# tphakala/birda

Hardware: AMD Instinct MI355X
Metric: 3s/48kHz segments/sec (BirdNET v2.4) (higher is better)
Workload: dtype f16x3; 1 GPU; configs[1]: 1000 synthetic 3 s/48 kHz segments per GPU per step, HBM-resident, seeded synthetic BirdNET-v2.4-shaped model (EfficientNet-B0-like, 6522 classes); segments_per_gpu=1000, micro_batch=1000, fused_blocks=16, precision=auto

## Files before the change

birda_amd/csrc/kernels_conv.hip:

```cpp
#include "kernels.hpp"

namespace bh {

typedef float f32x4 __attribute__((ext_vector_type(4)));

__device__ __forceinline__ float act_apply(float v, int act) { return act_apply_slow(v, act); }

constexpr int PW_BK = 32;

template <int BM, int NT, bool GATE = false>
__global__ __launch_bounds__(256) void pw_gemm_kernel(const float *__restrict__ A, const float *__restrict__ W,
                                                       const float *__restrict__ bias, const float *__restrict__ R,
                                                       float *__restrict__ C, int M, int K, int N, int ldw, int act,
                                                       const float *__restrict__ gate = nullptr, int rows_per_seg = 1, int res_after = 0) {
    constexpr int BN = NT * 16;
    constexpr int WM = BM / 4;
    constexpr int MT = WM / 16;
    constexpr int AS = PW_BK + 4;
    constexpr int BS = BN + 4;
    constexpr int A4 = BM * PW_BK / 4 / 256;
    constexpr int B4 = (PW_BK * BN / 4 + 255) / 256;
    __shared__ __attribute__((aligned(16))) float As[2][BM * AS];
    __shared__ __attribute__((aligned(16))) float Bs[2][PW_BK * BS];

// ... 255 lines not shown
    const int li = lane & 15, kq = lane >> 4;
    const int t0 = ((int)blockIdx.x * 4 + wave) * NT;
    if (t0 >= n_tiles) return;
    const int steps = K / 32;
    f32x4 acc[NT];
#pragma unroll
    for (int j = 0; j < NT; j++) acc[j] = (f32x4){0.f, 0.f, 0.f, 0.f};
    const float *arow = A + (size_t)min(li, M - 1) * K + 8 * kq;
    float4 ra[PF][2];
    f16x8 bh[PF][NT], bl[PF][NT];
    auto load = [&](int st, float4 (&a)[2], f16x8 (&h)[NT], f16x8 (&l)[NT]) {
        a[0] = *reinterpret_cast<const float4 *>(arow + 32 * st);
        a[1] = *reinterpret_cast<const float4 *>(arow + 32 * st + 4);
#pragma unroll
        for (int j = 0; j < NT; j++) {
            const int t = min(t0 + j, n_tiles - 1);
            h[j] = Wf[(((size_t)st * n_tiles + t) * BH_PL(TERMS) + 0) * 64 + lane];
            if (TERMS == 3) l[j] = Wf[(((size_t)st * n_tiles + t) * 2 + 1) * 64 + lane];
        }
    };
#pragma unroll
    for (int u = 0; u < PF; u++)
        if (u < steps) load(u, ra[u], bh[u], bl[u]);
    for (int st0 = 0; st0 < steps; st0 += PF) {
#pragma unroll
        for (int u = 0; u < PF; u++) {
            const int st = st0 + u;
            if (st < steps) {
                const float v[8] = {ra[u][0].x, ra[u][0].y, ra[u][0].z, ra[u][0].w, ra[u][1].x, ra[u][1].y, ra[u][1].z, ra[u][1].w};
                f16x8 ah, al;
                bh_split8(v, ah, al);
#pragma unroll
                for (int j = 0; j < NT; j++) {
                    acc[j] = __builtin_amdgcn_mfma_f32_16x16x32_f16(ah, bh[u][j], acc[j], 0, 0, 0);
                    if (TERMS == 3) acc[j] = __builtin_amdgcn_mfma_f32_16x16x32_f16(ah, bl[u][j], acc[j], 0, 0, 0);
                    if (TERMS >= 2) acc[j] = __builtin_amdgcn_mfma_f32_16x16x32_f16(al, bh[u][j], acc[j], 0, 0, 0);
                }
                if (st + PF < steps) load(st + PF, ra[u], bh[u], bl[u]);
            }
        }
    }
#pragma unroll
    for (int j = 0; j < NT; j++) {
        const int col = (t0 + j) * 16 + li;
        if (col >= N) continue;
        const float bv = bias[col];
#pragma unroll
        for (int r = 0; r < 4; r++) {
            const int row = kq * 4 + r;
            if (row < M) {
                float v = __builtin_fmaf(acc[j][r], w_unscale, bv);
                if constexpr (AFTER) v = bh_act_after<ACT>(v + R[(size_t)row * N + col]);
                else { v = bh_act<ACT>(v); if (R) v += R[(size_t)row * N + col]; }
                C[(size_t)row * N + col] = v;
            }
        }
    }
}

template <int TERMS, int ACT, bool GATE = false, int NTB = 8, bool BLK = false, bool AFTER = false>
__global__ __launch_bounds__(256, 2) void pw_gemm16s_kernel(const float *__restrict__ A, const f16x8 *__restrict__ Wf,
                                                            const float *__restrict__ bias, const float *__restrict__ R,
                                                            float *__restrict__ C, int M, int K, int N, int n_tiles, float w_unscale,
                                                            const float *__restrict__ gate = nullptr, int rows_per_seg = 1) {
    extern __shared__ __attribute__((aligned(16))) float gsm[];
    constexpr int STAGE = (8 + NTB) * 2 * 256;
    constexpr int NJ = NTB / 2;
    static_assert(NTB % 2 == 0 && NTB >= 2 && NTB <= 12, "column tiles per workgroup");
    static_assert(!(AFTER && GATE), "the gated project GEMMs have no after-the-add form");
    const int tid = threadIdx.x, lane = tid & 63, wave = tid >> 6;
    const int li = lane & 15, kq = lane >> 4;
    const int wm = wave >> 1, wn = wave & 1;
    const int n_xb = (n_tiles + NTB - 1) / NTB, n_yb = (M + 127) / 128;
    int yb, xb;
    if constexpr (GATE) {
        yb = (int)blockIdx.x / n_xb; xb = (int)blockIdx.x - yb * n_xb;
        if (yb >= n_yb) return;
    } else {
        const int xcd = blockIdx.x & 7, slot = blockIdx.x >> 3;
        yb = slot % n_yb; xb = (slot / n_yb) * 8 + xcd;
        if (xb >= n_xb) return;
    }
    const int mb0 = yb * 128, tb0 = xb * NTB;
    const int steps = GATE ? (K + 31) / 32 : K / 32;
    const unsigned lds0 = (__builtin_amdgcn_groupstaticsize() + 15u) & ~15u;
    const int ws = __builtin_amdgcn_readfirstlane(wave);

    const int srow = tid >> 2, skq = tid & 3;
    const float *ag[2], *gg[2];
    int adst[2];
#pragma unroll
    for (int q = 0; q < 2; q++) {
        const int row = srow + 64 * q, grow = min(mb0 + row, M - 1);
        ag[q] = BLK ? A + (size_t)(grow >> 4) * 16 * K + ((skq >> 1) * 16 + (grow & 15)) * 16 + (skq & 1) * 8 : A + (size_t)grow * K + 8 * skq;
        gg[q] = GATE ? gate + (size_t)(grow / rows_per_seg) * K + 8 * skq : nullptr;
        adst[q] = (((row >> 4) * 2) * 64 + skq * 16 + (row & 15)) * 4;
    }
    float4 ra[2][2], rg[GATE ? 2 : 1][2];
    constexpr int a_step = BLK ? 512 : 32;
    auto load_a = [&](int st) {
#pragma unroll
        for (int q = 0; q < 2; q++) {
            if constexpr (GATE) {
#pragma unroll
                for (int h = 0; h < 2; h++) {
                    const bool in = 32 * st + 8 * skq + 4 * h < K;
                    ra[q][h] = *reinterpret_cast<const float4 *>(ag[q] + (in ? a_step * st + 4 * h : 0));
                    rg[q][h] = *reinterpret_cast<const float4 *>(gg[q] + (in ? 32 * st + 4 * h : 0));
                    if (!in) { rg[q][h] = make_float4(0.f, 0.f, 0.f, 0.f); ra[q][h] = rg[q][h]; }
                }
            } else {
                ra[q][0] = *reinterpret_cast<const float4 *>(ag[q] + 32 * st);
                ra[q][1] = *reinterpret_cast<const float4 *>(ag[q] + 32 * st + 4);
            }
        }
    };
    auto store_a = [&](int buf) {
        float *as = gsm + buf * STAGE;
#pragma unroll
        for (int q = 0; q < 2; q++) {
            float v[8] = {ra[q][0].x, ra[q][0].y, ra[q][0].z, ra[q][0].w, ra[q][1].x, ra[q][1].y, ra[q][1].z, ra[q][1].w};
            if constexpr (GATE) {
                const float g[8] = {rg[q][0].x, rg[q][0].y, rg[q][0].z, rg[q][0].w, rg[q][1].x, rg[q][1].y, rg[q][1].z, rg[q][1].w};
#pragma unroll
                for (int j = 0; j < 8; j++) v[j] *= g[j];
            }
            f16x8 h, l;
            bh_split8(v, h, l);
            *reinterpret_cast<f16x8 *>(as + adst[q]) = h;
            if (TERMS >= 2) *reinterpret_cast<f16x8 *>(as + adst[q] + 256) = l;
        }
    };
    auto dma_b = [&](int st, int buf) {
#pragma unroll
        for (int jj = 0; jj < (NTB + 3) / 4; jj++) {
            const int j = ws + 4 * jj, t = min(tb0 + j, n_tiles - 1);
            if (j >= NTB) continue;
#pragma unroll
            for (int pl = 0; pl < (TERMS == 3 ? 2 : 1); pl++) {
                const f16x8 *src = Wf + (((size_t)st * n_tiles + t) * BH_PL(TERMS) + pl) * 64;
                const unsigned dst = lds0 + 4u * (unsigned)(buf * STAGE + 8 * 2 * 256 + (j * 2 + pl) * 256);
                asm volatile("s_mov_b32 m0, %2\n\ts_nop 0\n\tglobal_load_lds_dwordx4 %0, %1"
                             :: "v"((unsigned)lane * 16u), "s"(src), "s"(dst) : "memory", "m0");
            }
        }
    };

    f32x4 acc[4][NJ];
#pragma unroll
    for (int i = 0; i < 4; i++)
#pragma unroll
        for (int j = 0; j < NJ; j++) acc[i][j] = (f32x4){0.f, 0.f, 0.f, 0.f};

    dma_b(0, 0);
    load_a(0);
    store_a(0);
    asm volatile("s_waitcnt vmcnt(0)" ::: "memory");
    __syncthreads();
    for (int st = 0; st < steps; st++) {
        const int cur = st & 1;
        const bool more = st + 1 < steps;
        if (more) { dma_b(st + 1, cur ^ 1); load_a(st + 1); }
        const float *as = gsm + cur * STAGE, *bs = as + 8 * 2 * 256;
        f16x8 ah[4], al[4], bh[NJ], bl[NJ];
#pragma unroll
        for (int i = 0; i < 4; i++) {
            ah[i] = *reinterpret_cast<const f16x8 *>(as + (((wm * 4 + i) * 2) * 64 + lane) * 4);
            if (TERMS >= 2) al[i] = *reinterpret_cast<const f16x8 *>(as + (((wm * 4 + i) * 2 + 1) * 64 + lane) * 4);
        }
#pragma unroll
        for (int j = 0; j < NJ; j++) {
            bh[j] = *reinterpret_cast<const f16x8 *>(bs + (((wn * NJ + j) * 2) * 64 + lane) * 4);
            if (TERMS == 3) bl[j] = *reinterpret_cast<const f16x8 *>(bs + (((wn * NJ + j) * 2 + 1) * 64 + lane) * 4);
        }
#pragma unroll
        for (int i = 0; i < 4; i++)
#pragma unroll
            for (int j = 0; j < NJ; j++) {
                acc[i][j] = __builtin_amdgcn_mfma_f32_16x16x32_f16(ah[i], bh[j], acc[i][j], 0, 0, 0);
                if (TERMS == 3) acc[i][j] = __builtin_amdgcn_mfma_f32_16x16x32_f16(ah[i], bl[j], acc[i][j], 0, 0, 0);
                if (TERMS >= 2) acc[i][j] = __builtin_amdgcn_mfma_f32_16x16x32_f16(al[i], bh[j], acc[i][j], 0, 0, 0);
            }
        if (more) store_a(cur ^ 1);
        asm volatile("s_waitcnt vmcnt(0)" ::: "memory");
        __syncthreads();
    }
    const int m0 = mb0 + wm * 64, t0 = tb0 + wn * NJ;
#pragma unroll
    for (int j = 0; j < NJ; j++) {
        const int col = (t0 + j) * 16 + li;
        if (col >= N) continue;
        const float bv = bias[col];
#pragma unroll
        for (int i = 0; i < 4; i++)
#pragma unroll
            for (int r = 0; r < 4; r++) {
                const int row = m0 + i * 16 + kq * 4 + r;
                if (row < M) {
                    float v = __builtin_fmaf(acc[i][j][r], w_unscale, bv);
                    if constexpr (AFTER) v = bh_act_after<ACT>(v + R[(size_t)row * N + col]);
                    else { v = bh_act<ACT>(v); if (R) v += R[(size_t)row * N + col]; }
                    C[(size_t)row * N + col] = v;
                }
            }
    }
}

bool pw_gemm16_supports(int K, int act) { return K % 32 == 0 && (act == ACT_NONE || act_is_templated(act)); }
bool pw_gemm16_after_supports(int K, int act) { return K % 32 == 0 && act_is_templated_after(act); }

#define BH_LOAD_STREAM(p) (*(p))
template <int TERMS, int NT, bool SHALLOW = false, int DBG = 0>
__global__ __launch_bounds__(512, SHALLOW ? 4 : 2) void pw_gemm16_thin_kernel(const float *__restrict__ A, const float *__restrict__ gate, int rows_per_seg,
                                                                 const f16x8 *__restrict__ Wf, const float *__restrict__ bias,
                                                                 const float *__restrict__ R, float *__restrict__ C, int M, int K, int N,
                                                                 float w_unscale) {
    extern __shared__ __attribute__((aligned(16))) float tsm[];
    const int tid = threadIdx.x, lane = tid & 63, wave = tid >> 6;
    const int li = lane & 15, kq = lane >> 4;
    const int steps = (K + 31) / 32;
    {
        const float4 *src = reinterpret_cast<const float4 *>(Wf);
        float4 *dst = reinterpret_cast<float4 *>(tsm);
        const int n4 = steps * NT * BH_PL(TERMS) * 64;
        for (int i = tid; i < n4; i += 512) dst[i] = src[i];
    }
    __syncthreads();
    const f16x8 *wf = reinterpret_cast<const f16x8 *>(tsm);
    const int n_rt = (M + 15) >> 4;
    const float rcp_p = 1.0f / (float)rows_per_seg;
    constexpr int RB = SHALLOW ? (NT <= 2 ? 3 : 2) : (NT <= 2 ? 4 : 3);
    for (int rt0 = (blockIdx.x * 8 + wave) * RB; rt0 < n_rt; rt0 += gridDim.x * 8 * RB) {
        const float *ap[RB], *gp[RB];
#pragma unroll
        for (int r = 0; r < RB; r++) {
            const int row = min((rt0 + r) * 16 + li, M - 1);
            int seg = (int)((float)row * rcp_p);
            seg += (row - seg * rows_per_seg >= rows_per_seg) ? 1 : 0;
            seg -= (row - seg * rows_per_seg < 0) ? 1 : 0;
            ap[r] = A + (size_t)row * K + 8 * kq;
            gp[r] = gate + (size_t)seg * K + 8 * kq;
        }
        f32x4 acc[RB][NT];
#pragma unroll
        for (int r = 0; r < RB; r++)
#pragma unroll
            for (int j = 0; j < NT; j++) acc[r][j] = (f32x4){0.f, 0.f, 0.f, 0.f};
        float4 ra[RB][2], rg[RB][2];
        auto load = [&](int st, float4 (&a)[RB][2], float4 (&g)[RB][2]) {
#pragma unroll
            for (int r = 0; r < RB; r++)
#pragma unroll
                for (int h = 0; h < 2; h++) {
                    const bool in = 32 * st + 8 * kq + 4 * h < K;
                    a[r][h] = BH_LOAD_STREAM(reinterpret_cast<const float4 *>(ap[r] + (in ? 32 * st + 4 * h : 0)));
                    g[r][h] = *reinterpret_cast<const float4 *>(gp[r] + (in ? 32 * st + 4 * h : 0));
                    if (!in) { a[r][h] = make_float4(0.f, 0.f, 0.f, 0.f); g[r][h] = a[r][h]; }
                }
        };
        for (int st = 0; st < steps; st++) {
            load(st, ra, rg);
            f16x8 ah[RB], al[RB];
#pragma unroll
            for (int r = 0; r < RB; r++) {
                const float v[8] = {ra[r][0].x * rg[r][0].x, ra[r][0].y * rg[r][0].y, ra[r][0].z * rg[r][0].z, ra[r][0].w * rg[r][0].w,
                                    ra[r][1].x * rg[r][1].x, ra[r][1].y * rg[r][1].y, ra[r][1].z * rg[r][1].z, ra[r][1].w * rg[r][1].w};
                bh_split8(v, ah[r], al[r]);
            }
            if constexpr ((DBG & 1) != 0) {
#pragma unroll
                for (int r = 0; r < RB; r++) acc[r][0][0] += (float)ah[r][0] + (float)al[r][7];
                continue;
            }
#pragma unroll
            for (int j = 0; j < NT; j++) {
                const f16x8 bh = wf[((st * NT + j) * BH_PL(TERMS) + 0) * 64 + lane];
                f16x8 bl;
                if (TERMS == 3) bl = wf[((st * NT + j) * 2 + 1) * 64 + lane];
#pragma unroll
                for (int r = 0; r < RB; r++) {
                    acc[r][j] = __builtin_amdgcn_mfma_f32_16x16x32_f16(ah[r], bh, acc[r][j], 0, 0, 0);
                    if (TERMS == 3) acc[r][j] = __builtin_amdgcn_mfma_f32_16x16x32_f16(ah[r], bl, acc[r][j], 0, 0, 0);
                    if (TERMS >= 2) acc[r][j] = __builtin_amdgcn_mfma_f32_16x16x32_f16(al[r], bh, acc[r][j], 0, 0, 0);
                }
            }
        }
        if constexpr ((DBG & 8) != 0) {
            float t = 0.f;
#pragma unroll
            for (int r = 0; r < RB; r++)
#pragma unroll
                for (int j = 0; j < NT; j++) t += acc[r][j][0] + acc[r][j][1] + acc[r][j][2] + acc[r][j][3];
            if (t == 12345.678f) C[0] = t;
            continue;
        }
        float *ep = tsm + (size_t)steps * NT * BH_PL(TERMS) * 256 + (size_t)wave * (RB * 16 * NT * 16);
#pragma unroll
        for (int r = 0; r < RB; r++)
#pragma unroll
            for (int j = 0; j < NT; j++) {
                const int col = j * 16 + li;
                if (col >= N) continue;
                const float bv = bias[col];
#pragma unroll
                for (int q = 0; q < 4; q++) ep[(r * 16 + kq * 4 + q) * N + col] = __builtin_fmaf(acc[r][j][q], w_unscale, bv);
            }
        __builtin_amdgcn_fence(__ATOMIC_RELEASE, "wavefront");
        __builtin_amdgcn_wave_barrier();
        const int row0 = rt0 * 16, nrows = min(RB * 16, M - row0);
        const int nflt = nrows * N;
        float *cg = C + (size_t)row0 * N;
        const float *rgp = R ? R + (size_t)row0 * N : nullptr;
        for (int f = lane * 4; f < nflt; f += 256) {
            float4 v = *reinterpret_cast<const float4 *>(ep + f);
            if (rgp) { const float4 rr = *reinterpret_cast<const float4 *>(rgp + f); v.x += rr.x; v.y += rr.y; v.z += rr.z; v.w += rr.w; }
            *reinterpret_cast<float4 *>(cg + f) = v;
        }
        __builtin_amdgcn_wave_barrier();
    }
}

#define BH_GDBG(bit) ((DBG & (bit)) != 0)
template <int N_> __device__ __forceinline__ void bh_wait_vm() { asm volatile("s_waitcnt vmcnt(%0)" :: "n"(N_) : "memory"); }
template <int TERMS, int NT, int RB, int PF, int DBG = 0>
__global__ __launch_bounds__(512, 1) void pw_gemm16_wide_kernel(const float *__restrict__ A, const float *__restrict__ gate, int rows_per_seg,
                                                                 const f16x8 *__restrict__ Wf, const float *__restrict__ bias,
                                                                 const float *__restrict__ R, float *__restrict__ C, int M, int K, int N,
                                                                 float w_unscale, int gs_max, int a_blocked) {
    extern __shared__ __attribute__((aligned(16))) float wsm[];
    constexpr int PL = BH_PL(TERMS);
    constexpr int STEP_FL = NT * PL * 256;
    constexpr int PIECES = (NT * PL + 7) / 8;
    constexpr int ND = RB * 2;
    constexpr int INFLIGHT = ND + (PF - 2) * (PIECES + ND);
    static_assert(PF >= 2 && PF <= 4 && INFLIGHT <= 63, "prefetch depth");
    const int tid = threadIdx.x, lane = tid & 63, wave = tid >> 6;
    const int li = lane & 15, kq = lane >> 4;
    const int steps = (K + 31) / 32, KP = steps * 32;
    float *gs = wsm + PF * STEP_FL;
    float *ep = wsm + (size_t)wave * (16 * NT * 16);
    const int n_rt = (M + 15) >> 4;
    const float rcp_p = 1.0f / (float)rows_per_seg;
    const unsigned lds0 = (__builtin_amdgcn_groupstaticsize() + 15u) & ~15u;
    const int ws = __builtin_amdgcn_readfirstlane(wave);
    auto dma_w = [&](int st) {
        const int buf = st % PF;
#pragma unroll
        for (int i = 0; i < PIECES; i++) {
            const int p = min(ws + 8 * i, NT * PL - 1);
            const f16x8 *src = Wf + ((size_t)st * NT * PL + p) * 64;
            const unsigned dst = lds0 + 4u * (unsigned)(buf * STEP_FL + p * 256);
            asm volatile("s_mov_b32 m0, %2\n\ts_nop 0\n\tglobal_load_lds_dwordx4 %0, %1"
// ... 165 lines not shown
            asm volatile("" ::: "memory");
        }
        if constexpr (BH_GDBG(64)) {
            asm volatile("s_waitcnt vmcnt(0)" ::: "memory");
            const long long t_3 = __builtin_readcyclecounter();
            if (lane == 0) {
                long long *st = reinterpret_cast<long long *>(C + (size_t)M * N) + ((size_t)blockIdx.x * 8 + wave) * 4;
                st[0] = t_1 - t_0; st[1] = t_2 - t_1; st[2] = t_3 - t_2; st[3] = t_0;
            }
        }
    }
}

bool pw_gemm16_gated_wants_blocked(int K, int N, int rows_per_seg) {
    const int n_tiles = (N + 15) / 16;
    return K % 16 == 0 && rows_per_seg % 16 == 0 && N % 4 == 0 && n_tiles >= 6 && n_tiles <= 15;
}

const char *launch_pw_gemm16_gated(const float *A, const float *gate, int rows_per_seg, const void *Wf, const float *bias, const float *R,
                                   float *C, int M, int K, int N, int terms, float w_unscale, int a_blocked, hipStream_t s) {
    const char *name = nullptr;
    const int n_tiles = (N + 15) / 16;
    const size_t w_bytes = (size_t)((K + 31) / 32) * n_tiles * 2 * 1024;
    if (n_tiles <= 3 && w_bytes <= 64 * 1024 && M >= 4096 && N % 4 == 0 && !a_blocked) {
        const bool shallow = K <= 32;
        const size_t thin_lds = w_bytes / 2 * BH_PL(terms) + (size_t)8 * (shallow ? (n_tiles <= 2 ? 3 : 2) : (n_tiles <= 2 ? 4 : 3)) * 16 * n_tiles * 16 * sizeof(float);
        const int n_rt = (M + 15) / 16;
        const int wgs = std::min((n_rt + 31) / 32, 2 * device_cu_count());
#define BH_THIN(T, NTV, SH)                                                                                                        \
        do {                                                                                                                       \
            static DeviceOnce attr;                                                                                                \
            attr.run([] { (void)hipFuncSetAttribute((const void *)pw_gemm16_thin_kernel<T, NTV, SH>, hipFuncAttributeMaxDynamicSharedMemorySize, 128 * 1024); }); \
            hipLaunchKernelGGL((pw_gemm16_thin_kernel<T, NTV, SH>), dim3(wgs), dim3(512), thin_lds, s, A, gate, rows_per_seg, (const f16x8 *)Wf, bias, R, C, M, K, N, w_unscale); \
            name = "pw_gemm16_thin_kernel<" #T ",NT=" #NTV ",SHALLOW=" #SH ">";                                                   \
        } while (0)
#define BH_THIN_S(T, NTV) do { if (shallow) BH_THIN(T, NTV, true); else BH_THIN(T, NTV, false); } while (0)
        if (terms == 3) { if (n_tiles == 1) BH_THIN_S(3, 1); else if (n_tiles == 2) BH_THIN_S(3, 2); else BH_THIN_S(3, 3); }
        else if (terms == 2) { if (n_tiles == 1) BH_THIN_S(2, 1); else if (n_tiles == 2) BH_THIN_S(2, 2); else BH_THIN_S(2, 3); }
        else { if (n_tiles == 1) BH_THIN_S(1, 1); else if (n_tiles == 2) BH_THIN_S(1, 2); else BH_THIN_S(1, 3); }
#undef BH_THIN_S
#undef BH_THIN
        return name;
    }
    if (n_tiles >= 4 && n_tiles <= 15 && M >= (n_tiles >= 10 ? 40960 : 4096) && N % 4 == 0) {
        const int n_rt = (M + 15) / 16;
#define BH_WIDE(T, NTV, RBV, PFV)                                                                                                  \
        do {                                                                                                                       \
            const int gs_max = (8 * RBV * 16 + rows_per_seg - 2) / rows_per_seg + 1;                                              \
            const size_t lds = std::max((size_t)PFV * NTV * BH_PL(T) * 1024 + (size_t)gs_max * ((K + 31) / 32 * 32) * sizeof(float),         \
                                        (size_t)8 * 16 * NTV * 16 * sizeof(float));                                              \
            if (lds > 160 * 1024) break;                                \
            const int wgs = std::min((n_rt + 8 * RBV - 1) / (8 * RBV), device_cu_count());                                       \
            static DeviceOnce attr;                                                                                                \
            attr.run([] { (void)hipFuncSetAttribute((const void *)pw_gemm16_wide_kernel<T, NTV, RBV, PFV>, hipFuncAttributeMaxDynamicSharedMemorySize, 160 * 1024); }); \
            hipLaunchKernelGGL((pw_gemm16_wide_kernel<T, NTV, RBV, PFV>), dim3(wgs), dim3(512), lds, s, A, gate, rows_per_seg, (const f16x8 *)Wf, bias, R, C, M, K, N, w_unscale, gs_max, a_blocked); \
            return "pw_gemm16_wide_kernel<" #T ",NT=" #NTV ",RB=" #RBV ",PF=" #PFV ">";                                          \
        } while (0)
#define BH_WIDE_T(T)                                                                             \
        switch (n_tiles) {                                                                      \
        case 4: BH_WIDE(T, 4, 3, 3); break; case 5: BH_WIDE(T, 5, 3, 3); break; case 6: BH_WIDE(T, 6, 3, 3); break; case 7: BH_WIDE(T, 7, 3, 3); break; case 8: BH_WIDE(T, 8, 2, 4); break; case 9: BH_WIDE(T, 9, 2, 4); break;  \
        case 10: BH_WIDE(T, 10, 2, 3); break; case 11: BH_WIDE(T, 11, 2, 3); break; case 12: BH_WIDE(T, 12, 2, 3); break; case 13: BH_WIDE(T, 13, 2, 3); break; \
        case 14: BH_WIDE(T, 14, 2, 3); break; default: BH_WIDE(T, 15, 2, 3); break; }
        if (terms == 3) { BH_WIDE_T(3) } else if (terms == 2) { BH_WIDE_T(2) } else { BH_WIDE_T(1) }
#undef BH_WIDE_T
#undef BH_WIDE
    }
    int ntb = 8;
    {
        long best = -1;
        for (int cand : {10, 8, 6}) {
            const long padded = (long)((n_tiles + cand - 1) / cand) * cand;
            if (best < 0 || padded < best) { best = padded; ntb = cand; }
        }
    }
    const int n_xb = (n_tiles + ntb - 1) / ntb, n_yb = (M + 127) / 128;
    dim3 grid((unsigned)(n_xb * n_yb)), block(256);
#define BH_GS(T, NTBV, BLKV)                                                                                                      \
    do {                                                                                                                          \
        constexpr size_t lds = 2 * ((8 + NTBV) * 2 * 256) * sizeof(float);                                                       \
        static DeviceOnce attr;                                                                                                   \
        attr.run([] { (void)hipFuncSetAttribute((const void *)pw_gemm16s_kernel<T, ACT_NONE, true, NTBV, BLKV>, hipFuncAttributeMaxDynamicSharedMemorySize, (int)lds); }); \
        hipLaunchKernelGGL((pw_gemm16s_kernel<T, ACT_NONE, true, NTBV, BLKV>), grid, block, lds, s, A, (const f16x8 *)Wf, bias, R, C, M, K, N, n_tiles, w_unscale, gate, rows_per_seg); \
        name = "pw_gemm16s_kernel<" #T ",NONE,GATE,NTB=" #NTBV ",BLK=" #BLKV ">";                                                 \
    } while (0)
#define BH_GS_B(T, NTBV) do { if (a_blocked) BH_GS(T, NTBV, true); else BH_GS(T, NTBV, false); } while (0)
    if (terms == 3) { if (ntb == 6) BH_GS_B(3, 6); else if (ntb == 10) BH_GS_B(3, 10); else BH_GS_B(3, 8); }
    else if (terms == 2) { if (ntb == 6) BH_GS_B(2, 6); else if (ntb == 10) BH_GS_B(2, 10); else BH_GS_B(2, 8); }
    else { if (ntb == 6) BH_GS_B(1, 6); else if (ntb == 10) BH_GS_B(1, 10); else BH_GS_B(1, 8); }
#undef BH_GS_B
#undef BH_GS
    return name;
}

const char *launch_pw_gemm16(const float *A, const void *Wf, const float *bias, const float *R, float *C, int M, int K, int N,
                             int act, int terms, float w_unscale, hipStream_t s, int res_after) {
    if (res_after && (!R || !act_is_templated_after(act))) return nullptr;
    const int n_tiles = (N + 15) / 16;
    const int n_xb = (n_tiles + 7) / 8, n_yb = (M + 127) / 128;
    dim3 grid((unsigned)(8 * ((n_xb + 7) / 8) * n_yb)), block(256);
    static const bool stream_only = [] { const char *e = BH_XENV("BIRDA_HIP_GEMM_STREAM"); return e && e[0] == '1'; }();
    const bool staged = M >= 64 && !stream_only;
    const int ntb = !staged ? 8 : n_xb * n_yb >= 384 ? 8 : ((n_tiles + 3) / 4) * n_yb >= 384 ? 4 : 2;
    const int n_xb_s = (n_tiles + ntb - 1) / ntb;
    const dim3 grid_s((unsigned)(8 * ((n_xb_s + 7) / 8) * n_yb));
    const char *name = nullptr;
#define BH_G16S(T, ACTV, AN, NTBV, AFT, AFN)                                                                                      \
    do {                                                                                                                          \
        constexpr size_t lds = 2 * ((8 + NTBV) * 2 * 256) * sizeof(float);                                                        \
        static DeviceOnce attr;                                                                                                   \
        attr.run([] { (void)hipFuncSetAttribute((const void *)pw_gemm16s_kernel<T, ACTV, false, NTBV, false, AFT>, hipFuncAttributeMaxDynamicSharedMemorySize, (int)lds); }); \
        hipLaunchKernelGGL((pw_gemm16s_kernel<T, ACTV, false, NTBV, false, AFT>), grid_s, block, lds, s, A, (const f16x8 *)Wf, bias, R, C, M, K, N, n_tiles, w_unscale); \
        name = "pw_gemm16s_kernel<" #T "," AN AFN ",NTB=" #NTBV ">";                                                             \
    } while (0)
#define BH_G16(T, ACTV, AN, AFT, AFN)                                                                                             \
    do {                                                                                                                          \
        if (staged) {                                                                                                             \
            if (ntb == 8) BH_G16S(T, ACTV, AN, 8, AFT, AFN); else if (ntb == 4) BH_G16S(T, ACTV, AN, 4, AFT, AFN); else BH_G16S(T, ACTV, AN, 2, AFT, AFN); \
        } else if (M <= 32) {     \
            for (int m0 = 0; m0 < M; m0 += 16)                                                                                    \
                hipLaunchKernelGGL((pw_gemm16_skinny_kernel<T, ACTV, AFT>), dim3((unsigned)((n_tiles + 7) / 8)), block, 0, s, A + (size_t)m0 * K, (const f16x8 *)Wf, bias, \
                                   R ? R + (size_t)m0 * N : nullptr, C + (size_t)m0 * N, std::min(16, M - m0), K, N, n_tiles, w_unscale); \
            name = "pw_gemm16_skinny_kernel<" #T "," AN AFN ">";                                                                 \
        } else {                                                                                                                  \
            hipLaunchKernelGGL((pw_gemm16_kernel<T, ACTV, AFT>), grid, block, 0, s, A, (const f16x8 *)Wf, bias, R, C, M, K, N, n_tiles, w_unscale); \
            name = "pw_gemm16_kernel<" #T "," AN AFN ">";                                                                        \
        }                                                                                                                         \
    } while (0)
#define BH_G16A(T)                                                   \
    switch (act) {                                                   \
    case ACT_GELU_ERF: BH_G16(T, ACT_GELU_ERF, "GELU", false, ""); break; \
    case ACT_SWISH: BH_G16(T, ACT_SWISH, "SWISH", false, ""); break; \
    case ACT_RELU6: BH_G16(T, ACT_RELU6, "RELU6", false, ""); break; \
    case ACT_HSWISH: BH_G16(T, ACT_HSWISH, "HSWISH", false, ""); break; \
    default: BH_G16(T, ACT_NONE, "NONE", false, ""); break;          \
    }
#define BH_G16AA(T)                                                  \
    switch (act) {                                                   \
    case ACT_GELU_ERF: BH_G16(T, ACT_GELU_ERF, "GELU", true, ",AFTER"); break; \
    case ACT_SWISH: BH_G16(T, ACT_SWISH, "SWISH", true, ",AFTER"); break; \
    case ACT_RELU6: BH_G16(T, ACT_RELU6, "RELU6", true, ",AFTER"); break; \
    case ACT_HSWISH: BH_G16(T, ACT_HSWISH, "HSWISH", true, ",AFTER"); break; \
    default: BH_G16(T, ACT_RELU, "RELU", true, ",AFTER"); break;     \
    }
    if (res_after) { if (terms == 3) { BH_G16AA(3) } else if (terms == 2) { BH_G16AA(2) } else { BH_G16AA(1) } }
    else if (terms == 3) { BH_G16A(3) } else if (terms == 2) { BH_G16A(2) } else { BH_G16A(1) }
#undef BH_G16AA
#undef BH_G16A
#undef BH_G16
#undef BH_G16S
    return name;
}

template <int PT, int SW, int TERMS, int ACT, int CT = 8>
__global__ __launch_bounds__(256, 1) void head_gap16_kernel(const float *__restrict__ A, const f16x8 *__restrict__ Wf,
                                                             const float *__restrict__ bias, float *__restrict__ out,
                                                             int n_seg, int P, int K, int N, int n_tiles, int n_cb, float w_unscale) {
    constexpr int RT = PT * SW;
    constexpr int PL = BH_PL(TERMS);
    __shared__ __attribute__((aligned(16))) f16x8 Bs[2][CT * PL * 64];
    const int tid = threadIdx.x, lane = tid & 63, wave = tid >> 6;
    const int li = lane & 15, kq = lane >> 4;
    const int xcd = blockIdx.x & 7, bi = blockIdx.x >> 3;
    const int cb = bi % n_cb, mb = (bi / n_cb) * 8 + xcd;
    const int seg0 = (mb * 4 + wave) * SW;
    if (mb * 4 * SW >= n_seg) return;
    const int steps = K / 32;

    auto dma = [&](int st, int buf) {
        const f16x8 *src = Wf + ((size_t)st * n_tiles + cb * CT) * PL * 64;
#pragma unroll
        for (int q = 0; q < (CT * PL + 3) / 4; q++) {
            const int piece = q * 4 + wave;
            if (piece >= CT * PL) continue;
            const unsigned la = (unsigned)(size_t)(&Bs[buf][piece * 64]);
            asm volatile("s_mov_b32 m0, %1\n\ts_nop 0\n\tglobal_load_lds_dwordx4 %0, off"
                         :: "v"(src + piece * 64 + lane), "s"(__builtin_amdgcn_readfirstlane(la)) : "memory", "m0");
        }
    };
    int aoff[RT];
#pragma unroll
    for (int i = 0; i < RT; i++) {
        const int seg = min(seg0 + i / PT, n_seg - 1), px = min((i % PT) * 16 + li, P - 1);
        aoff[i] = (seg * P + px) * K + 8 * kq;
    }
    float4 ra[RT][2];
    auto load_a = [&](int st) {
#pragma unroll
        for (int i = 0; i < RT; i++) {
            ra[i][0] = *reinterpret_cast<const float4 *>(A + (size_t)aoff[i] + 32 * st);
            ra[i][1] = *reinterpret_cast<const float4 *>(A + (size_t)aoff[i] + 32 * st + 4);
        }
    };
    f32x4 acc[RT][CT];
#pragma unroll
    for (int j = 0; j < CT; j++)
#pragma unroll
        for (int i = 0; i < RT; i++) acc[i][j] = (f32x4){0.f, 0.f, 0.f, 0.f};
    f16x8 ah[RT], al[RT];
    auto split_a = [&]() {
#pragma unroll
        for (int i = 0; i < RT; i++) {
            const float v[8] = {ra[i][0].x, ra[i][0].y, ra[i][0].z, ra[i][0].w, ra[i][1].x, ra[i][1].y, ra[i][1].z, ra[i][1].w};
            bh_split8(v, ah[i], al[i]);
        }
    };
    auto compute = [&](int buf) {
#pragma unroll
        for (int j = 0; j < CT; j++) {
            const f16x8 bh = Bs[buf][(j * PL + 0) * 64 + lane];
            f16x8 bl;
            if (TERMS == 3) bl = Bs[buf][(j * 2 + 1) * 64 + lane];
#pragma unroll
            for (int i = 0; i < RT; i++) {
                acc[i][j] = __builtin_amdgcn_mfma_f32_16x16x32_f16(ah[i], bh, acc[i][j], 0, 0, 0);
                if (TERMS == 3) acc[i][j] = __builtin_amdgcn_mfma_f32_16x16x32_f16(ah[i], bl, acc[i][j], 0, 0, 0);
                if (TERMS >= 2) acc[i][j] = __builtin_amdgcn_mfma_f32_16x16x32_f16(al[i], bh, acc[i][j], 0, 0, 0);
            }
        }
    };
    dma(0, 0);
    load_a(0);
    asm volatile("s_waitcnt vmcnt(0)" ::: "memory");
    __syncthreads();
    for (int st = 0; st + 1 < steps; st++) {
        dma(st + 1, (st + 1) & 1);
        split_a();
        __builtin_amdgcn_sched_barrier(0);
        load_a(st + 1);
        __builtin_amdgcn_sched_barrier(0);
        compute(st & 1);
        asm volatile("s_waitcnt vmcnt(0)" ::: "memory");
        __syncthreads();
    }
    split_a();
    __builtin_amdgcn_sched_barrier(0);
    compute((steps - 1) & 1);

    const float inv_p = 1.0f / (float)P;
#pragma unroll
    for (int sg = 0; sg < SW; sg++) {
        const int seg = seg0 + sg;
#pragma unroll
        for (int j = 0; j < CT; j++) {
            float sum = 0.0f;
            const float b = bias[(cb * CT + j) * 16 + li];
#pragma unroll
            for (int t = 0; t < PT; t++) {
                const f32x4 a4 = acc[sg * PT + t][j];
                bh_f32x2 v01 = {__builtin_fmaf(a4[0], w_unscale, b), __builtin_fmaf(a4[1], w_unscale, b)},
                         v23 = {__builtin_fmaf(a4[2], w_unscale, b), __builtin_fmaf(a4[3], w_unscale, b)};
                bh_act4<ACT>(v01, v23);
                const int px = t * 16 + 4 * kq;
                if (PT * 16 == P || px + 3 < P) sum += (v01[0] + v01[1]) + (v23[0] + v23[1]);
                else sum += (px < P ? v01[0] : 0.f) + (px + 1 < P ? v01[1] : 0.f) + (px + 2 < P ? v23[0] : 0.f);
            }
            sum += __shfl_xor(sum, 16, 64);
            sum += __shfl_xor(sum, 32, 64);
            if (kq == 0 && seg < n_seg) out[(size_t)seg * N + (cb * CT + j) * 16 + li] = sum * inv_p;
        }
    }
}

bool head_gap16_supports(int P, int K, int N, int act) {
    return act_is_templated(act) && K % 32 == 0 && N % 128 == 0 && P >= 1 && P <= 80;
}

const char *launch_head_gap16(const float *A, const void *Wf, const float *bias, float *out, int n_seg, int P, int K, int N,
                              int act, int terms, float w_unscale, hipStream_t s) {
    const bool few = n_seg <= 32;
    const int n_tiles = N / 16, n_cb = few ? N / 32 : N / 128;
    const int pt = (P + 15) / 16, sw = pt <= 3 ? 2 : 1;
    const int n_mb = (n_seg + 4 * sw - 1) / (4 * sw);
    dim3 grid((unsigned)(((n_mb + 7) / 8) * n_cb * 8)), block(256);
    const char *name = nullptr;
#define BH_HG(PTV, SWV, T, ACTV, AN) do { if (few) hipLaunchKernelGGL((head_gap16_kernel<PTV, SWV, T, ACTV, 2>), grid, block, 0, s, A, (const f16x8 *)Wf, bias, out, \
                                                    n_seg, P, K, N, n_tiles, n_cb, w_unscale); \
    else hipLaunchKernelGGL((head_gap16_kernel<PTV, SWV, T, ACTV, 8>), grid, block, 0, s, A, (const f16x8 *)Wf, bias, out, \
                                                    n_seg, P, K, N, n_tiles, n_cb, w_unscale); \
    name = few ? "head_gap16_kernel<PT=" #PTV ",SW=" #SWV ",T=" #T "," AN ",CT=2>" : "head_gap16_kernel<PT=" #PTV ",SW=" #SWV ",T=" #T "," AN ",CT=8>"; } while (0)
#define BH_HGA(PTV, SWV, T)                                          \
    switch (act) {                                                   \
    case ACT_SWISH: BH_HG(PTV, SWV, T, ACT_SWISH, "SWISH"); break;   \
    case ACT_RELU6: BH_HG(PTV, SWV, T, ACT_RELU6, "RELU6"); break;   \
    case ACT_HSWISH: BH_HG(PTV, SWV, T, ACT_HSWISH, "HSWISH"); break;   \
    default: BH_HG(PTV, SWV, T, ACT_GELU_ERF, "GELU"); break;        \
    }
    if (pt <= 3) { if (terms == 3) { BH_HGA(3, 2, 3) } else if (terms == 2) { BH_HGA(3, 2, 2) } else { BH_HGA(3, 2, 1) } }
    else { if (terms == 3) { BH_HGA(5, 1, 3) } else if (terms == 2) { BH_HGA(5, 1, 2) } else { BH_HGA(5, 1, 1) } }
#undef BH_HGA
#undef BH_HG
    return name;
}

template <int KS, int ST>
__global__ __launch_bounds__(256) void dwconv_kernel(const float *__restrict__ in, const float *__restrict__ w,
                                                      const float *__restrict__ b, float *__restrict__ out,
                                                      ConvParams p, int n_seg) {
    const int c4n = p.cout >> 2;
    const long total = (long)n_seg * p.out_h * p.out_w * c4n;
    for (long g = (long)blockIdx.x * 256 + threadIdx.x; g < total; g += (long)gridDim.x * 256) {
        const int c4 = (int)(g % c4n);
        long px = g / c4n;
        const int ox = (int)(px % p.out_w);
        px /= p.out_w;
        const int oy = (int)(px % p.out_h);
        const int seg = (int)(px / p.out_h);
        const int c = c4 << 2;
        float4 acc = *reinterpret_cast<const float4 *>(b + c);
        const float *ib = in + (size_t)seg * p.in_h * p.in_w * p.cout + c;
        const int iy0 = oy * ST - p.pad_t, ix0 = ox * ST - p.pad_l;
#pragma unroll
        for (int dy = 0; dy < KS; dy++) {
            const int iy = iy0 + dy;
            if (iy < 0 || iy >= p.in_h) continue;
#pragma unroll
            for (int dx = 0; dx < KS; dx++) {
                const int ix = ix0 + dx;
                if (ix < 0 || ix >= p.in_w) continue;
                const float4 a = *reinterpret_cast<const float4 *>(ib + ((size_t)iy * p.in_w + ix) * p.cout);
                const float4 ww = *reinterpret_cast<const float4 *>(w + (size_t)(dy * KS + dx) * p.cout + c);
                acc.x += a.x * ww.x; acc.y += a.y * ww.y; acc.z += a.z * ww.z; acc.w += a.w * ww.w;
            }
        }
        acc.x = act_apply(acc.x, p.act); acc.y = act_apply(acc.y, p.act);
        acc.z = act_apply(acc.z, p.act); acc.w = act_apply(acc.w, p.act);
        *reinterpret_cast<float4 *>(out + (((size_t)seg * p.out_h + oy) * p.out_w + ox) * p.cout + c) = acc;
    }
}

bool dwconv_supports(const ConvParams &p) {
    return p.cout % 4 == 0 && p.kh == p.kw && p.sh == p.sw && (p.kh == 3 || p.kh == 5) && (p.sh == 1 || p.sh == 2);
}

const char *launch_dwconv(const float *in, const float *w, const float *b, float *out, const ConvParams &p, int n_seg,
                          hipStream_t s) {
    const long total = (long)n_seg * p.out_h * p.out_w * (p.cout / 4);
    long blocks = (total + 255) / 256;
    if (blocks > 256L * 64) blocks = 256L * 64;
    dim3 grid((unsigned)blocks), block(256);
#define BH_DW_CASE(KSV, STV)                                                                       \
    if (p.kh == KSV && p.sh == STV) {                                                               \
        hipLaunchKernelGGL((dwconv_kernel<KSV, STV>), grid, block, 0, s, in, w, b, out, p, n_seg);  \
        return "dwconv_kernel<" #KSV "," #STV ">";                                                  \
    }
    BH_DW_CASE(3, 1) BH_DW_CASE(3, 2) BH_DW_CASE(5, 1) BH_DW_CASE(5, 2)
#undef BH_DW_CASE
    return nullptr;
}

template <int NC>
__global__ __launch_bounds__(256) void conv_direct_kernel(const float *__restrict__ in, const float *__restrict__ w,
                                                           const float *__restrict__ b, float *__restrict__ out,
                                                           ConvParams p, int n_seg) {
    extern __shared__ __attribute__((aligned(16))) float ws[];
    const int wn = p.kh * p.kw * p.cin * p.cout;
    for (int i = threadIdx.x; i < wn; i += 256) ws[i] = w[i];
    __syncthreads();
    const int cgn = p.cout / NC;
    const long total = (long)n_seg * p.out_h * p.out_w * cgn;
    for (long g = (long)blockIdx.x * 256 + threadIdx.x; g < total; g += (long)gridDim.x * 256) {
        const int cg = (int)(g % cgn);
        long px = g / cgn;
        const int ox = (int)(px % p.out_w);
        px /= p.out_w;
        const int oy = (int)(px % p.out_h);
        const int seg = (int)(px / p.out_h);
        const int co = cg * NC;
        float acc[NC];
#pragma unroll
        for (int n = 0; n < NC; n++) acc[n] = b[co + n];
        const float *ib = in + (size_t)seg * p.in_h * p.in_w * p.cin;
        for (int dy = 0; dy < p.kh; dy++) {
            const int iy = oy * p.sh - p.pad_t + dy;
            if (iy < 0 || iy >= p.in_h) continue;
            for (int dx = 0; dx < p.kw; dx++) {
                const int ix = ox * p.sw - p.pad_l + dx;
                if (ix < 0 || ix >= p.in_w) continue;
                for (int c = 0; c < p.cin; c++) {
                    const float a = p.in_layout == 1 ? ib[((size_t)c * p.in_h + iy) * p.in_w + ix]
                                                     : ib[((size_t)iy * p.in_w + ix) * p.cin + c];
                    const float *wr = ws + ((dy * p.kw + dx) * p.cin + c) * p.cout + co;
#pragma unroll
                    for (int n = 0; n < NC; n++) acc[n] += a * wr[n];
                }
            }
        }
        float *o = out + (((size_t)seg * p.out_h + oy) * p.out_w + ox) * p.cout + co;
#pragma unroll
        for (int q = 0; q < NC; q += 4)
            *reinterpret_cast<float4 *>(o + q) = make_float4(act_apply(acc[q], p.act), act_apply(acc[q + 1], p.act), act_apply(acc[q + 2], p.act),
                                                             act_apply(acc[q + 3], p.act));
    }
}

bool conv_direct_supports(const ConvParams &p) {
    return p.cout % 4 == 0 && (size_t)p.kh * p.kw * p.cin * p.cout * sizeof(float) <= 64 * 1024;
}

const char *launch_conv_direct(const float *in, const float *w, const float *b, float *out, const ConvParams &p,
                               int n_seg, hipStream_t s) {
    if (!conv_direct_supports(p)) return nullptr;
    const int nc = p.cout % 8 ? 4 : 8;
    const long total = (long)n_seg * p.out_h * p.out_w * (p.cout / nc);
    long blocks = (total + 255) / 256;
    if (blocks > 256L * 32) blocks = 256L * 32;
    const size_t smem = (size_t)p.kh * p.kw * p.cin * p.cout * sizeof(float);
    if (nc == 8) hipLaunchKernelGGL(conv_direct_kernel<8>, dim3((unsigned)blocks), dim3(256), smem, s, in, w, b, out, p, n_seg);
    else hipLaunchKernelGGL(conv_direct_kernel<4>, dim3((unsigned)blocks), dim3(256), smem, s, in, w, b, out, p, n_seg);
    return nc == 8 ? "conv_direct_kernel<NC=8>" : "conv_direct_kernel<NC=4>";
}

// ... 736 lines not shown
```

Measured before the change: 153,600 segments/s.

## Split head GAP kernel into per-segment passes and peel GEMM pipeline loop

The head GEMM+GAP kernel with CT=8 now processes its SW segments in sequential passes, each holding accumulators for one segment. This lowers register pressure, and the launch bound asks for SW blocks per CU. The next pass's A/B loads are issued before the current pass's epilogue. B fragments in the compute loop are double-buffered, and sched barriers separate LDS reads from MFMAs. The fp16 pointwise GEMM also peels its last iteration, hoists the bias loads and fences the compute phase. The pass loop repeats the weight DMA per pass, so weight traffic grows in exchange for occupancy.

```diff
diff --git a/birda_amd/csrc/kernels_conv.hip b/birda_amd/csrc/kernels_conv.hip
--- a/birda_amd/csrc/kernels_conv.hip
+++ b/birda_amd/csrc/kernels_conv.hip
@@ -431,52 +431,62 @@
 #pragma unroll
         for (int j = 0; j < NJ; j++) acc[i][j] = (f32x4){0.f, 0.f, 0.f, 0.f};
 
+    const int m0 = mb0 + wm * 64, t0 = tb0 + wn * NJ;
+    float bv[NJ];
+#pragma unroll
+    for (int j = 0; j < NJ; j++) bv[j] = bias[min((t0 + j) * 16 + li, N - 1)];
+
+    auto compute = [&](int cur) {
+        const float *as = gsm + cur * STAGE, *bs = as + 8 * 2 * 256;
+        f16x8 ah[4], al[4], bh[NJ], bl[NJ];
+#pragma unroll
+        for (int i = 0; i < 4; i++) {
+            ah[i] = *reinterpret_cast<const f16x8 *>(as + (((wm * 4 + i) * 2) * 64 + lane) * 4);
+            if (TERMS >= 2) al[i] = *reinterpret_cast<const f16x8 *>(as + (((wm * 4 + i) * 2 + 1) * 64 + lane) * 4);
+        }
+#pragma unroll
+        for (int j = 0; j < NJ; j++) {
+            bh[j] = *reinterpret_cast<const f16x8 *>(bs + (((wn * NJ + j) * 2) * 64 + lane) * 4);
+            if (TERMS == 3) bl[j] = *reinterpret_cast<const f16x8 *>(bs + (((wn * NJ + j) * 2 + 1) * 64 + lane) * 4);
+        }
+        __builtin_amdgcn_sched_barrier(0);
+#pragma unroll
+        for (int i = 0; i < 4; i++)
+#pragma unroll
+            for (int j = 0; j < NJ; j++) {
+                acc[i][j] = __builtin_amdgcn_mfma_f32_16x16x32_f16(ah[i], bh[j], acc[i][j], 0, 0, 0);
+                if (TERMS == 3) acc[i][j] = __builtin_amdgcn_mfma_f32_16x16x32_f16(ah[i], bl[j], acc[i][j], 0, 0, 0);
+                if (TERMS >= 2) acc[i][j] = __builtin_amdgcn_mfma_f32_16x16x32_f16(al[i], bh[j], acc[i][j], 0, 0, 0);
+            }
+        __builtin_amdgcn_sched_barrier(0);
+    };
+
     dma_b(0, 0);
     load_a(0);
     store_a(0);
     asm volatile("s_waitcnt vmcnt(0)" ::: "memory");
     __syncthreads();
-    for (int st = 0; st < steps; st++) {
+    for (int st = 0; st + 1 < steps; st++) {
         const int cur = st & 1;
-        const bool more = st + 1 < steps;
-        if (more) { dma_b(st + 1, cur ^ 1); load_a(st + 1); }
-        const float *as = gsm + cur * STAGE, *bs = as + 8 * 2 * 256;
-        f16x8 ah[4], al[4], bh[NJ], bl[NJ];
-#pragma unroll
-        for (int i = 0; i < 4; i++) {
-            ah[i] = *reinterpret_cast<const f16x8 *>(as + (((wm * 4 + i) * 2) * 64 + lane) * 4);
-            if (TERMS >= 2) al[i] = *reinterpret_cast<const f16x8 *>(as + (((wm * 4 + i) * 2 + 1) * 64 + lane) * 4);
-        }
-#pragma unroll
-        for (int j = 0; j < NJ; j++) {
-            bh[j] = *reinterpret_cast<const f16x8 *>(bs + (((wn * NJ + j) * 2) * 64 + lane) * 4);
-            if (TERMS == 3) bl[j] = *reinterpret_cast<const f16x8 *>(bs + (((wn * NJ + j) * 2 + 1) * 64 + lane) * 4);
-        }
-#pragma unroll
-        for (int i = 0; i < 4; i++)
-#pragma unroll
-            for (int j = 0; j < NJ; j++) {
-                acc[i][j] = __builtin_amdgcn_mfma_f32_16x16x32_f16(ah[i], bh[j], acc[i][j], 0, 0, 0);
-                if (TERMS == 3) acc[i][j] = __builtin_amdgcn_mfma_f32_16x16x32_f16(ah[i], bl[j], acc[i][j], 0, 0, 0);
-                if (TERMS >= 2) acc[i][j] = __builtin_amdgcn_mfma_f32_16x16x32_f16(al[i], bh[j], acc[i][j], 0, 0, 0);
-            }
-        if (more) store_a(cur ^ 1);
+        dma_b(st + 1, cur ^ 1);
+        load_a(st + 1);
+        compute(cur);
+        store_a(cur ^ 1);
         asm volatile("s_waitcnt vmcnt(0)" ::: "memory");
         __syncthreads();
     }
-    const int m0 = mb0 + wm * 64, t0 = tb0 + wn * NJ;
+    compute((steps - 1) & 1);
 #pragma unroll
     for (int j = 0; j < NJ; j++) {
         const int col = (t0 + j) * 16 + li;
         if (col >= N) continue;
-        const float bv = bias[col];
 #pragma unroll
         for (int i = 0; i < 4; i++)
 #pragma unroll
             for (int r = 0; r < 4; r++) {
                 const int row = m0 + i * 16 + kq * 4 + r;
                 if (row < M) {
-                    float v = __builtin_fmaf(acc[i][j][r], w_unscale, bv);
+                    float v = __builtin_fmaf(acc[i][j][r], w_unscale, bv[j]);
                     if constexpr (AFTER) v = bh_act_after<ACT>(v + R[(size_t)row * N + col]);
                     else { v = bh_act<ACT>(v); if (R) v += R[(size_t)row * N + col]; }
                     C[(size_t)row * N + col] = v;
@@ -948,10 +958,11 @@
 }
 
 template <int PT, int SW, int TERMS, int ACT, int CT = 8>
-__global__ __launch_bounds__(256, 1) void head_gap16_kernel(const float *__restrict__ A, const f16x8 *__restrict__ Wf,
+__global__ __launch_bounds__(256, CT == 8 ? SW : 1) void head_gap16_kernel(const float *__restrict__ A, const f16x8 *__restrict__ Wf,
                                                              const float *__restrict__ bias, float *__restrict__ out,
                                                              int n_seg, int P, int K, int N, int n_tiles, int n_cb, float w_unscale) {
-    constexpr int RT = PT * SW;
+    constexpr int NP = CT == 8 ? SW : 1, SP = SW / NP;
+    constexpr int RT = PT * SP;
     constexpr int PL = BH_PL(TERMS);
     __shared__ __attribute__((aligned(16))) f16x8 Bs[2][CT * PL * 64];
     const int tid = threadIdx.x, lane = tid & 63, wave = tid >> 6;
@@ -974,11 +985,13 @@
         }
     };
     int aoff[RT];
-#pragma unroll
-    for (int i = 0; i < RT; i++) {
-        const int seg = min(seg0 + i / PT, n_seg - 1), px = min((i % PT) * 16 + li, P - 1);
-        aoff[i] = (seg * P + px) * K + 8 * kq;
-    }
+    auto rows_of = [&](int pass) {
+#pragma unroll
+        for (int i = 0; i < RT; i++) {
+            const int seg = min(seg0 + pass * SP + i / PT, n_seg - 1), px = min((i % PT) * 16 + li, P - 1);
+            aoff[i] = (seg * P + px) * K + 8 * kq;
+        }
+    };
     float4 ra[RT][2];
     auto load_a = [&](int st) {
 #pragma unroll
@@ -988,10 +1001,6 @@
         }
     };
     f32x4 acc[RT][CT];
-#pragma unroll
-    for (int j = 0; j < CT; j++)
-#pragma unroll
-        for (int i = 0; i < RT; i++) acc[i][j] = (f32x4){0.f, 0.f, 0.f, 0.f};
     f16x8 ah[RT], al[RT];
     auto split_a = [&]() {
 #pragma unroll
@@ -1001,58 +1010,81 @@
         }
     };
     auto compute = [&](int buf) {
+        f16x8 bh[2], bl[2];
+        bh[0] = Bs[buf][lane];
+        if (TERMS == 3) bl[0] = Bs[buf][64 + lane];
 #pragma unroll
         for (int j = 0; j < CT; j++) {
-            const f16x8 bh = Bs[buf][(j * PL + 0) * 64 + lane];
-            f16x8 bl;
-            if (TERMS == 3) bl = Bs[buf][(j * 2 + 1) * 64 + lane];
+            if (j + 1 < CT) {
+                bh[(j + 1) & 1] = Bs[buf][((j + 1) * PL + 0) * 64 + lane];
+                if (TERMS == 3) bl[(j + 1) & 1] = Bs[buf][((j + 1) * 2 + 1) * 64 + lane];
+            }
+            __builtin_amdgcn_sched_barrier(0);
 #pragma unroll
             for (int i = 0; i < RT; i++) {
-                acc[i][j] = __builtin_amdgcn_mfma_f32_16x16x32_f16(ah[i], bh, acc[i][j], 0, 0, 0);
-                if (TERMS == 3) acc[i][j] = __builtin_amdgcn_mfma_f32_16x16x32_f16(ah[i], bl, acc[i][j], 0, 0, 0);
-                if (TERMS >= 2) acc[i][j] = __builtin_amdgcn_mfma_f32_16x16x32_f16(al[i], bh, acc[i][j], 0, 0, 0);
-            }
+                acc[i][j] = __builtin_amdgcn_mfma_f32_16x16x32_f16(ah[i], bh[j & 1], acc[i][j], 0, 0, 0);
+                if (TERMS == 3) acc[i][j] = __builtin_amdgcn_mfma_f32_16x16x32_f16(ah[i], bl[j & 1], acc[i][j], 0, 0, 0);
+                if (TERMS >= 2) acc[i][j] = __builtin_amdgcn_mfma_f32_16x16x32_f16(al[i], bh[j & 1], acc[i][j], 0, 0, 0);
+            }
+            __builtin_amdgcn_sched_barrier(0);
         }
     };
+    float bv[CT];
+#pragma unroll
+    for (int j = 0; j < CT; j++) bv[j] = bias[(cb * CT + j) * 16 + li];
+    const float inv_p = 1.0f / (float)P;
+    rows_of(0);
     dma(0, 0);
     load_a(0);
-    asm volatile("s_waitcnt vmcnt(0)" ::: "memory");
-    __syncthreads();
-    for (int st = 0; st + 1 < steps; st++) {
-        dma(st + 1, (st + 1) & 1);
+#pragma unroll
+    for (int pass = 0; pass < NP; pass++) {
+#pragma unroll
+        for (int j = 0; j < CT; j++)
+#pragma unroll
+            for (int i = 0; i < RT; i++) acc[i][j] = (f32x4){0.f, 0.f, 0.f, 0.f};
+        asm volatile("s_waitcnt vmcnt(0)" ::: "memory");
+        __syncthreads();
+        for (int st = 0; st + 1 < steps; st++) {
+            split_a();
+            __builtin_amdgcn_sched_barrier(0);
+            dma(st + 1, (st + 1) & 1);
+            load_a(st + 1);
+            __builtin_amdgcn_sched_barrier(0);
+            compute(st & 1);
+            asm volatile("s_waitcnt vmcnt(0)" ::: "memory");
+            __syncthreads();
+        }
         split_a();
         __builtin_amdgcn_sched_barrier(0);
-        load_a(st + 1);
-        __builtin_amdgcn_sched_barrier(0);
-        compute(st & 1);
-        asm volatile("s_waitcnt vmcnt(0)" ::: "memory");
-        __syncthreads();
-    }
-    split_a();
-    __builtin_amdgcn_sched_barrier(0);
-    compute((steps - 1) & 1);
-
-    const float inv_p = 1.0f / (float)P;
-#pragma unroll
-    for (int sg = 0; sg < SW; sg++) {
-        const int seg = seg0 + sg;
-#pragma unroll
-        for (int j = 0; j < CT; j++) {
-            float sum = 0.0f;
-            const float b = bias[(cb * CT + j) * 16 + li];
-#pragma unroll
-            for (int t = 0; t < PT; t++) {
-                const f32x4 a4 = acc[sg * PT + t][j];
-                bh_f32x2 v01 = {__builtin_fmaf(a4[0], w_unscale, b), __builtin_fmaf(a4[1], w_unscale, b)},
-                         v23 = {__builtin_fmaf(a4[2], w_unscale, b), __builtin_fmaf(a4[3], w_unscale, b)};
-                bh_act4<ACT>(v01, v23);
-                const int px = t * 16 + 4 * kq;
-                if (PT * 16 == P || px + 3 < P) sum += (v01[0] + v01[1]) + (v23[0] + v23[1]);
-                else sum += (px < P ? v01[0] : 0.f) + (px + 1 < P ? v01[1] : 0.f) + (px + 2 < P ? v23[0] : 0.f);
-            }
-            sum += __shfl_xor(sum, 16, 64);
-            sum += __shfl_xor(sum, 32, 64);
-            if (kq == 0 && seg < n_seg) out[(size_t)seg * N + (cb * CT + j) * 16 + li] = sum * inv_p;
+        compute((steps - 1) & 1);
+        if (pass + 1 < NP) {
+            __syncthreads();
+            rows_of(pass + 1);
+            dma(0, 0);
+            load_a(0);
+        }
+
+#pragma unroll
+        for (int sg = 0; sg < SP; sg++) {
+            const int seg = seg0 + pass * SP + sg;
+#pragma unroll
+            for (int j = 0; j < CT; j++) {
+                float sum = 0.0f;
+                const float b = bv[j];
+#pragma unroll
+                for (int t = 0; t < PT; t++) {
+                    const f32x4 a4 = acc[sg * PT + t][j];
+                    bh_f32x2 v01 = {__builtin_fmaf(a4[0], w_unscale, b), __builtin_fmaf(a4[1], w_unscale, b)},
+                             v23 = {__builtin_fmaf(a4[2], w_unscale, b), __builtin_fmaf(a4[3], w_unscale, b)};
+                    bh_act4<ACT>(v01, v23);
+                    const int px = t * 16 + 4 * kq;
+                    if (PT * 16 == P || px + 3 < P) sum += (v01[0] + v01[1]) + (v23[0] + v23[1]);
+                    else sum += (px < P ? v01[0] : 0.f) + (px + 1 < P ? v01[1] : 0.f) + (px + 2 < P ? v23[0] : 0.f);
+                }
+                sum += __shfl_xor(sum, 16, 64);
+                sum += __shfl_xor(sum, 32, 64);
+                if (kq == 0 && seg < n_seg) out[(size_t)seg * N + (cb * CT + j) * 16 + li] = sum * inv_p;
+            }
         }
     }
 }
```

After: 154,600 segments/s, median of 6. No clear change (+0.6%).
